# bkomuves/plonky2-verifier

Measured on AMD Instinct MI355X. Metric: Plonky2 proofs verified/sec (std config, 28 FRI queries) at 1/2/4/8 MI355X, higher is better.
Workload: dtype u64 (Goldilocks mod-p integer)

## Files before the change

### plonky2-verifier_amd/csrc/api_selftest.cpp

```cpp
#include "api_internal.hpp"
#include "kernels.h"

extern "C" {

static int selftest_field(int op, const uint64_t* a, const uint64_t* b, uint64_t* out, size_t n) {
  static const size_t kB[9] = {0, 0, 0, 0, 0, 1, 1, 12, 1}, kIn[9] = {2, 4, 1, 2, 4, 1, 2, 0, 0}, kOut[9] = {5, 2, 1, 2, 4, 1, 2, 2, 2};
  const size_t bw = kB[op - 12], wo = kOut[op - 12];
  size_t w = kIn[op - 12];
  if (bw && !b) return fail(P2V_E_ARG, "bad op / null argument");
  if (op == 17 && b[0] > 32) return fail(P2V_E_ARG, "pow_root: k > 32");
  if (op == 18 && b[0] > 0xFFFFFFFFull) return fail(P2V_E_ARG, "epow_u: e >= 2^32");
  if (op == 19) {
    w = (size_t)b[0];
    bool ok = b[0] >= 2 && b[0] <= (1u << 20) && b[1] <= 5;
    for (int k = 0; k < 5 && ok; k++) ok = b[2 + k] <= b[0] && b[7 + k] <= b[0] - b[2 + k];
    if (!ok) return fail(P2V_E_ARG, "reduce_powers: segment table outside the item");
  }
  if (op == 20) {
    if (b[0] < 1 || b[0] > 8) return fail(P2V_E_ARG, "fold: arity bits outside 1..8");
    w = 2 + (2u << b[0]);
  }
  if (n > (size_t)INT32_MAX - 64) return fail(P2V_E_ARG, "too many items");
  if (n == 0) return P2V_OK;
  Circuit C;
  C.arities = {1, 2, 3, 4, 5, 6, 7, 8};
  C.step_depth.assign(8, 0); C.L.step_evals.assign(8, 0); C.L.step_path.assign(8, 0);
  DevCircuit d{};
  fill_scalars(C, d);
  DevBuf da, db, dout, dtw;
#define SCK(x) HCK_AS("p2v_selftest", x)
  SCK(da.alloc(n * w * 8)); SCK(db.alloc(bw * 8)); SCK(dout.alloc(n * wo * 8));
  SCK(upload(dtw, fri_twiddles(C), d.twiddles));
  SCK(hipMemcpy(da.p, a, n * w * 8, hipMemcpyHostToDevice));
  if (bw) SCK(hipMemcpy(db.p, b, bw * 8, hipMemcpyHostToDevice));
  d.soa = (const uint64_t*)da.p; d.words = (int64_t)w; d.wstride = 1; d.tiled = 0;
  d.n = (int32_t)n; d.B = (int32_t)((n + 63) / 64 * 64);
  hipLaunchKernelGGL(k_selftest_field, dim3((unsigned)((n + 255) / 256)), dim3(256), 0, 0, op, d, (const uint64_t*)db.p, (uint64_t*)dout.p);
  SCK(hipGetLastError());
  SCK(hipMemcpy(out, dout.p, n * wo * 8, hipMemcpyDeviceToHost));
#undef SCK
  return P2V_OK;
}

static int selftest_prog(int device, const uint64_t* a, const uint64_t* b, uint64_t* out, size_t n) {
  if (!b) return fail(P2V_E_ARG, "bad op / null argument");
  if (b[0] > (1u << 20) || b[1] > (1u << 20)) return fail(P2V_E_ARG, "gate program rows beyond this build's limits");
  if (n > (size_t)INT32_MAX - 64) return fail(P2V_E_ARG, "too many items");
  const int64_t nw = (int64_t)b[0], nc = (int64_t)b[1];
  GateProgram g;
  std::vector<uint64_t> low;
  try {
    if (b[2] != P2V_WORDS_GATE_MAGIC) throw ParseError("gate program: bad magic / version");
    if (b[3] > (uint64_t)P2V_GATE_PROGRAM_MAX_INSTRS) throw CircuitError("gate program beyond this build's limits (instructions)");
    g = decode_gate_program(b + 2, gate_program_extent(b + 2, 2 + 3 * (size_t)b[3]));
    if (g.max_wire >= nw || g.max_const >= nc) throw CircuitError("(Array.!): gate program reads beyond the row");
    if (g.max_pih >= 4) throw CircuitError("(!!): gate program reads a public-inputs-hash word beyond 4");
    if (lower_gate_program(g, &low) > P2V_GATE_PROGRAM_MAX_LIVE) throw CircuitError("gate program beyond this build's limits (values alive at once)");
  } catch (const std::exception& e) { return fail(P2V_E_ARG, std::string("selftest op 21: ") + e.what()); }
  const int ndev = p2v_device_count();
  if (ndev == 0) return fail(P2V_E_NODEVICE, "no HIP device");
  if (device < 0 || device >= ndev) return fail(P2V_E_ARG, "bad device index");
  if (n == 0 || g.num_commits == 0) return P2V_OK;
  HCK(hipSetDevice(device));
  const size_t w = (size_t)(2 * (nw + nc) + 4), wo = 2 * (size_t)g.num_commits;
  DevCircuit d{};
  d.prog_pih = 2 * (nw + nc);
  d.o_wires = 0; d.o_const = 2 * nw;
  d.words = (int64_t)w; d.wstride = 1; d.tiled = 0;
  d.n = (int32_t)n; d.B = (int32_t)((n + 63) / 64 * 64);
  DevBuf da, dout, dprog;
#define SCK(x) HCK_AS("p2v_selftest", x)
  SCK(da.alloc(n * w * 8)); SCK(dout.alloc(n * wo * 8));
  SCK(upload(dprog, low, d.gprog));
  SCK(hipMemcpy(da.p, a, n * w * 8, hipMemcpyHostToDevice));
  d.soa = (const uint64_t*)da.p;
  hipLaunchKernelGGL(k_selftest_prog, dim3((unsigned)((n + 63) / 64)), dim3(64), 0, 0, d, (uint64_t*)dout.p, g.num_commits);
  SCK(hipGetLastError());
  SCK(hipMemcpy(out, dout.p, n * wo * 8, hipMemcpyDeviceToHost));
#undef SCK
  return P2V_OK;
}

int p2v_selftest(int device, int op, const uint64_t* a, const uint64_t* b, uint64_t* out, size_t n) {
  const bool needs_b = op == 0 || op == 3 || op == 4 || op == 6;
  if (op < 0 || op > 21 || op == 11 || (n && (!a || !out || (needs_b && !b)))) return fail(P2V_E_ARG, "bad op / null argument");
  if (op == 21) return selftest_prog(device, a, b, out, n);
  const int ndev = p2v_device_count();
  if (ndev == 0) return fail(P2V_E_NODEVICE, "no HIP device");
  if (device < 0 || device >= ndev) return fail(P2V_E_ARG, "bad device index");
  if (op < 12 && n == 0) return P2V_OK;
  HCK(hipSetDevice(device));
  if (op >= 12) return selftest_field(op, a, b, out, n);
  const bool scalar = op == 0 || op == 3 || op == 5 || op == 6 || op == 7 || op == 8;
  const size_t w = scalar ? 1 : 12, wo = op == 6 ? 2 : w;
  const size_t bw = op == 4 ? 24 : scalar && needs_b ? n : 2;
  DevBuf da, db, dout;
#define SCK(x) HCK_AS("p2v_selftest", x)
  SCK(da.alloc(n * w * 8)); SCK(db.alloc(bw * 8)); SCK(dout.alloc(n * wo * 8));
  SCK(hipMemcpy(da.p, a, n * w * 8, hipMemcpyHostToDevice));
  if (needs_b) SCK(hipMemcpy(db.p, b, bw * 8, hipMemcpyHostToDevice));
  if (op >= 9) {
    const int lanes = op == 9 ? 16 : 4;
    hipLaunchKernelGGL(k_selftest_forms, dim3((unsigned)((n * lanes + 255) / 256)), dim3(256), 0, 0, op, (const uint64_t*)da.p,
                       (uint64_t*)dout.p, (int64_t)n);
  } else {
    const size_t lanes = op == 8 ? 2 : 1;
    hipLaunchKernelGGL(k_selftest, dim3((unsigned)((n * lanes + 255) / 256)), dim3(256), 0, 0, op, (const uint64_t*)da.p,
                       (const uint64_t*)db.p, (uint64_t*)dout.p, (int64_t)n);
  }
  SCK(hipGetLastError());
  SCK(hipMemcpy(out, dout.p, n * wo * 8, hipMemcpyDeviceToHost));
#undef SCK
  return P2V_OK;
}

int p2v_count_mismatches(const int8_t* results, const int8_t* expect, size_t n, uint64_t* counters, void* stream) {
  if (!counters || (n && (!results || !expect))) return fail(P2V_E_ARG, "null argument");
  const unsigned blocks = n ? (unsigned)((n + 255) / 256) : 1;
  hipLaunchKernelGGL(k_count_mismatches, dim3(blocks), dim3(256), 0, (hipStream_t)stream, results, expect, (int64_t)n,
                     (unsigned long long*)counters);
  HCK(hipGetLastError());
  return P2V_OK;
}

int p2v_clock_probe(uint64_t* stamps, int nblocks, void* stream) {
  if (!stamps || nblocks <= 0) return fail(P2V_E_ARG, "null argument / no blocks");
  hipLaunchKernelGGL(k_clock_probe, dim3((unsigned)nblocks), dim3(64), 0, (hipStream_t)stream, (unsigned long long*)stamps);
  HCK(hipGetLastError());
  return P2V_OK;
}

}
```

### plonky2-verifier_amd/csrc/kernels.hip

```cpp
#include "leafhash.h"
#include "kernels.h"

using namespace p2d;
using gl::E;

__device__ __forceinline__ void leaf_hash_unit(const DevCircuit& c, int unit, int lane) {
  const int NPB = c.B >> 6;
  const int pb = unit % NPB, qt = unit / NPB;
  const int q = qt % c.Q, t = c.leaf_order[qt / c.Q];
  const int p = pb * 64 + lane;
  const int64_t base = c.q0 + (int64_t)q * c.qstride;
  int64_t off; int len;
  if (t < 4) { off = base + c.leaf[t]; len = c.lwidth[t]; }
  else { int s = t - 4; off = base + c.step_evals[s]; len = 2 << c.arity[s]; }
  uint64_t st[12];
  leaf_sponge(c, off, len, p, st);
  uint64_t* dst = c.leafdig + ((int64_t)(q * c.T + t) * 4) * c.B + p;
#pragma unroll
  for (int i = 0; i < 4; i++) dst[(int64_t)i * c.B] = st[i];
}

template <int D>
__device__ __forceinline__ uint64_t row_up(uint64_t v, bool plus) {
  const uint32_t lo = (uint32_t)v, hi = (uint32_t)(v >> 32);
// ... 461 lines not shown
  const bool pow_ok = (resp & mask) == 0;
  int8_t st = 1;
  if (!eqs_ok || !pow_ok) st = 0;
  else {
    for (int q = 0; q < c.Q && st == 1; q++) {
      const uint8_t* mk = c.mk_ok + (int64_t)q * c.T * c.B + p;
      bool init_ok = mk[0] && mk[c.B] && mk[2 * (int64_t)c.B] && mk[3 * (int64_t)c.B];
      if (!init_ok) { st = -1; break; }
      const uint32_t bits = c.fri_bits[(int64_t)q * c.B + p];
      for (int s = 0; s < c.S; s++) {
        if (!mk[(int64_t)(4 + s) * c.B]) { st = -2; break; }
        if (!((bits >> s) & 1u)) { st = -3; break; }
      }
      if (st != 1) break;
      if (!((bits >> 31) & 1u)) st = 0;
    }
  }
  if (c.key_id && c.key_id[p] >= (uint32_t)c.nkeys) st = -6;
  results[p] = st;
  if (trace) {
    uint64_t* tr = trace + (int64_t)p * trace_words;
    const int r = c.r, S = c.S, Q = c.Q;
    int64_t k = 0;
    for (int64_t w = 0; w < CH_QIDX(c) + Q; w++) tr[k++] = chal(c, w, p);
    for (int i = 0; i < 4 * r; i++) tr[k++] = c.van[(int64_t)(1 + i) * c.B + p];
    for (int j = 0; j < 3; j++)
      for (int q = 0; q < Q; q++) {
        const uint64_t* qv = c.qvals + (int64_t)q * 6 * c.B + p;
        tr[k++] = qv[(int64_t)(2 * j) * c.B];
        tr[k++] = qv[(int64_t)(2 * j + 1) * c.B];
      }
    tr[k++] = (uint64_t)(eqs_ok ? 1 : 0) | ((uint64_t)(pow_ok ? 1 : 0) << 1);
    for (int i = 0; i < r * c.nluts; i++) tr[k++] = c.lutre[(int64_t)i * c.B + p];
    (void)S;
  }
}

extern "C" __global__ void __launch_bounds__(256) k_selftest(int op, const uint64_t* a, const uint64_t* b, uint64_t* out, int64_t n) {
  const int64_t i = (int64_t)blockIdx.x * blockDim.x + threadIdx.x;
  if (op == 8) {
#if defined(__HIP_DEVICE_COMPILE__)
    const int64_t item = i >> 1;
    const uint64_t x = lp::sbox_u(a[item < n ? item : n - 1], (int)(i & 1));
    if (item < n && !(i & 1)) out[item] = gl::canon(x);
#endif
    return;
  }
  if (i >= n) return;
  if (op >= 5 && op <= 7) {
#if defined(__HIP_DEVICE_COMPILE__)
    if (op == 5) { uint64_t x = a[i]; p2::dv::sbox_n<1>(&x); out[i] = gl::canon(x); }
    else if (op == 6) { uint64_t x[2] = {a[i], b[i]}; p2::dv::sbox_n<2>(x); out[2 * i] = gl::canon(x[0]); out[2 * i + 1] = gl::canon(x[1]); }
    else out[i] = gl::canon(lp::sbox(a[i]));
#endif
  } else if (op == 0) {
    out[i] = gl::mul(a[i], b[i]);
  } else if (op == 3) {
#if defined(__HIP_DEVICE_COMPILE__)
    out[i] = gl::canon(gl::mul_nc_dev_v<2>(a[i], b[i]));
#endif
  } else if (op == 4) {
#if defined(__HIP_DEVICE_COMPILE__)
    uint64_t st[12], t[12], kl[12], kh[12];
#pragma unroll
    for (int k = 0; k < 12; k++) { st[k] = a[12 * i + k]; kl[k] = b[k]; kh[k] = b[12 + k]; }
    p2::dv::mds_group<0>(st, t, kl, kh);
    p2::dv::mds_group<4>(st, t, kl, kh);
    p2::dv::mds_group<8>(st, t, kl, kh);
#pragma unroll
    for (int k = 0; k < 12; k++) out[12 * i + k] = t[k];
#endif
  } else {
    uint64_t s[12];
#pragma unroll
    for (int k = 0; k < 12; k++) s[k] = op == 2 && k >= 8 ? 0 : a[12 * i + k];
    if (op == 1) p2::permute_dev(s);
    else p2::permute_dev(s, true, 1);
#pragma unroll
    for (int k = 0; k < 12; k++) out[12 * i + k] = op == 2 && k >= 4 ? 0 : s[k];
  }
}

extern "C" __global__ void __launch_bounds__(256) k_selftest_forms(int op, const uint64_t* a, uint64_t* out, int64_t n) {
  __shared__ TLdsAny T;
  tlds_fill_form(T, op == 9 ? 16 : 4);
  const int lanes = op == 9 ? 16 : 4;
  const int64_t g = (int64_t)blockIdx.x * 256 + threadIdx.x;
  const int64_t item = g / lanes, src = item < n ? item : n - 1;
  const int t = (int)(g % lanes);
  const uint64_t* s = a + 12 * src;
  uint64_t* o = out + 12 * item;
  if (op == 9) {
    lp::Row LR;
    lp::init(LR, T.l, threadIdx.x);
    const uint64_t x = lp::permute(LR.L < 12 ? s[LR.L] : 0, LR, T.l);
    if (item < n && LR.L < 12) o[LR.L] = x;
  } else {
    uint64_t x[3] = {s[3 * t], s[3 * t + 1], s[3 * t + 2]};
    qp::permute(x, t, T.q);
    if (item < n) for (int k = 0; k < 3; k++) o[3 * t + k] = x[k];
  }
}

extern "C" __global__ void __launch_bounds__(256) k_selftest_field(int op, DevCircuit c, const uint64_t* b, uint64_t* out) {
  const int64_t i = (int64_t)blockIdx.x * blockDim.x + threadIdx.x;
  const int p = (int)i;
  const bool live = i < c.n;
  if (op == 12) {
    const uint64_t x = ld(c, 0, p), y = ld(c, 1, p);
    const uint64_t r[5] = {gl::add(x, y), gl::sub(x, y), gl::neg(x), gl::mul_small(x, 7), gl::mul_small(x, (uint32_t)y)};
    if (live) for (int k = 0; k < 5; k++) out[5 * i + k] = r[k];
  } else if (op == 13) {
    const E x = lde(c, 0, p), y = lde(c, 2, p);
    const E r = gl::eeq(x, y) ? gl::esqr(x) : gl::emul(x, y);
    if (live) { out[2 * i] = r.a; out[2 * i + 1] = r.b; }
  } else if (op == 14) {
    const uint64_t r = inv_chain(ld(c, 0, p));
    if (live) out[i] = r;
  } else if (op == 15) {
    const E r = einv(lde(c, 0, p));
    if (live) { out[2 * i] = r.a; out[2 * i + 1] = r.b; }
  } else if (op == 16) {
    E iu, iv;
    einv2(lde(c, 0, p), lde(c, 2, p), iu, iv);
    if (live) { out[4 * i] = iu.a; out[4 * i + 1] = iu.b; out[4 * i + 2] = iv.a; out[4 * i + 3] = iv.b; }
  } else if (op == 17) {
    const uint64_t r = pow_root(c, (int)b[0], (uint32_t)ld(c, 0, p));
    if (live) out[i] = r;
  } else if (op == 18) {
    const E r = epow_u(lde(c, 0, p), (uint32_t)b[0]);
    if (live) { out[2 * i] = r.a; out[2 * i + 1] = r.b; }
  } else if (op == 19) {
    Segs S;
    S.ns = (int)b[1];
    for (int k = 0; k < 5; k++) { S.off[k] = (int64_t)b[2 + k]; S.n[k] = (int)b[7 + k]; }
    const E alpha = lde(c, 0, p);
    E ap[9];
    alpha_powers(alpha, ap);
    const E r = reduce_powers(c, S, p, alpha, ap);
    if (live) { out[2 * i] = r.a; out[2 * i + 1] = r.b; }
  } else if (op == 20) {
    const int ab = (int)b[0];
    const E r = fold_step(c, ab - 1, ab, 2, p, lde(c, 0, p));
    if (live) { out[2 * i] = r.a; out[2 * i + 1] = r.b; }
  }
}
```

### plonky2-verifier_amd/csrc/merkle.hip

```cpp
#include "leafhash.h"
#include "kernels.h"

using namespace p2d;

__device__ __forceinline__ uint32_t entry_pack(int t, int q, int p) { return (uint32_t)t << 27 | (uint32_t)q << 22 | (uint32_t)p; }
__device__ __forceinline__ void entry_unpack(uint32_t id, int& t, int& q, int& p) {
  t = (int)(id >> 27); q = (int)((id >> 22) & 31); p = (int)(id & 0x3FFFFFu);
}
__device__ __forceinline__ uint32_t plan_pack(int e, int owner, bool same_leaf, int root) {
  return (uint32_t)e | (uint32_t)owner << 4 | (uint32_t)same_leaf << 9 | (uint32_t)root << 10;
}
__device__ __forceinline__ int plan_e(uint32_t pw) { return (int)(pw & 15); }
__device__ __forceinline__ int plan_owner(uint32_t pw) { return (int)((pw >> 4) & 31); }
__device__ __forceinline__ bool plan_same_leaf(uint32_t pw) { return (pw >> 9) & 1; }
__device__ __forceinline__ int plan_root(uint32_t pw) { return (int)((pw >> 10) & 31); }
__device__ __forceinline__ uint8_t& mk_at(const DevCircuit& c, int t, int q, int p) { return c.mk_ok[(int64_t)(q * c.T + t) * c.B + p]; }

#ifndef P2V_MERKLE_WAVES
#define P2V_MERKLE_WAVES 6
#endif
#if P2V_MERKLE_WAVES > 0
#define P2V_MERKLE_ATTR __attribute__((amdgpu_waves_per_eu(P2V_MERKLE_WAVES)))
#else
#define P2V_MERKLE_ATTR
#endif
__device__ __forceinline__ void tree_path(const DevCircuit& c, int t, int q, int p, int& depth, int64_t& poff, uint32_t& idx) {
  const int64_t base = c.q0 + (int64_t)q * c.qstride;
  idx = (uint32_t)chal(c, CH_QIDX(c) + q, p);
  if (t < 4) { depth = c.depth0; poff = base + c.path[t]; }
  else {
    const int s = t - 4;
    int sh = 0;
    for (int j = 0; j <= s; j++) sh += c.arity[j];
    idx >>= sh; depth = c.step_depth[s]; poff = base + c.step_path[s];
  }
}
__device__ __forceinline__ void load_leafdig(const DevCircuit& c, int t, int q, int p, uint64_t (&cur)[4]) {
  const uint64_t* src = c.leafdig + ((int64_t)(q * c.T + t) * 4) * c.B + p;
#pragma unroll
  for (int i = 0; i < 4; i++) cur[i] = src[(int64_t)i * c.B];
}
__device__ __forceinline__ uint64_t cap_root(const DevCircuit& c, int t, uint32_t ci, int i, int p) {
  if (t == 0) return c.key_id ? lane_key(c, p)[ci * 4 + i] : c.cs_cap[ci * 4 + i];
  if (t == 1) return ld(c, c.wcap + ci * 4 + i, p);
  if (t == 2) return ld(c, c.zcap + ci * 4 + i, p);
  if (t == 3) return ld(c, c.qcap + ci * 4 + i, p);
  return ld(c, c.ccaps + (int64_t)(t - 4) * 4 * c.cap_len + ci * 4 + i, p);
}

__device__ __forceinline__ void merkle_level(uint64_t (&cur)[4], const uint64_t (&sib)[4], bool odd) {
  uint64_t st[12];
#pragma unroll
  for (int i = 0; i < 4; i++) { st[i] = odd ? sib[i] : cur[i]; st[4 + i] = odd ? cur[i] : sib[i]; st[8 + i] = 0; }
  p2::permute_dev(st, true, 1);
#pragma unroll
  for (int i = 0; i < 4; i++) cur[i] = st[i];
}
struct NoNode { __device__ __forceinline__ void operator()(int) const {} };
template <class F = NoNode>
__device__ __forceinline__ void lane_climb(const DevCircuit& c, int64_t poff, int l0, int l1, int p, uint64_t (&cur)[4], uint32_t& idx, F node = F{}) {
  for (int l = l0; l < l1; l++) {
    uint64_t sib[4];
#pragma unroll
    for (int i = 0; i < 4; i++) sib[i] = ld(c, poff + 4 * l + i, p);
    node(l);
    merkle_level(cur, sib, idx & 1u);
    idx >>= 1;
  }
}
__device__ __forceinline__ bool cap_ok(const DevCircuit& c, int t, uint32_t idx, const uint64_t (&cur)[4], int p) {
  bool ok = idx < (uint32_t)c.cap_len;
  const uint32_t ci = ok ? idx : 0;
#pragma unroll
  for (int i = 0; i < 4; i++) ok = ok && (cap_root(c, t, ci, i, p) == cur[i]);
  return ok;
}

__device__ __forceinline__ uint64_t row_climb(const DevCircuit& c, int64_t poff, int l0, int depth, int p, const lp::Row& LR, const lp::TLdsL& TL,
                                              uint64_t cur, uint32_t& idx) {
  const int L = LR.L;
  for (int l = l0; l < depth; l++) {
    const uint64_t sib = L < 8 ? ld(c, poff + 4 * l + (L & 3), p) : 0;
    const uint64_t c0 = rp::get_word(cur, 0), c1 = rp::get_word(cur, 1), c2 = rp::get_word(cur, 2), c3 = rp::get_word(cur, 3);
    const uint64_t cb = L == 4 ? c0 : L == 5 ? c1 : L == 6 ? c2 : c3;
    const bool odd = idx & 1u;
    const uint64_t x = L < 4 ? (odd ? sib : cur) : L < 8 ? (odd ? cb : sib) : 0;
    cur = lp::permute(x, LR, TL);
    idx >>= 1;
  }
  return cur;
}
__device__ __forceinline__ bool row_cap_ok(const DevCircuit& c, int t, uint32_t idx, uint64_t cur, int p, int L) {
  const bool ok = idx < (uint32_t)c.cap_len;
  const uint32_t ci = ok ? idx : 0;
  uint64_t root = 0;
  if (L < 4) root = cap_root(c, t, ci, L, p);
  const uint64_t eq = (L >= 4 || root == cur) ? 1 : 0;
  return ok && (rp::get_word(eq, 0) & rp::get_word(eq, 1) & rp::get_word(eq, 2) & rp::get_word(eq, 3));
}

__device__ __forceinline__ bool path_ok(const DevCircuit& c, int t, int q, int p) {
  int depth; int64_t poff; uint32_t idx;
  tree_path(c, t, q, p, depth, poff, idx);
  uint64_t cur[4];
  load_leafdig(c, t, q, p, cur);
  lane_climb(c, poff, 0, depth, p, cur, idx);
  return cap_ok(c, t, idx, cur, p);
}
__device__ __forceinline__ void merkle_unit(const DevCircuit& c) {
  const int lane = threadIdx.x & 63;
  const int unit = blockIdx.x * 4 + (threadIdx.x >> 6);
  const int NPB = c.B >> 6;
  if (unit >= c.Q * c.T * NPB) return;
  const int pb = unit % NPB, qt = unit / NPB;
  const int q = qt % c.Q, t = c.merkle_order[qt / c.Q];
  const int p = pb * 64 + lane;
  mk_at(c, t, q, p) = path_ok(c, t, q, p) ? 1 : 0;
}
extern "C" __global__ void __launch_bounds__(256) P2V_MERKLE_ATTR k_merkle(DevCircuit c) { merkle_unit(c); }

#define P2V_CSE_CSTRIDE 16
__device__ __forceinline__ void class_shape(const DevCircuit& c, int cls, int& sh, int& depth) {
  sh = 0; depth = c.depth0;
  if (cls > 0) { for (int j = 0; j < cls; j++) sh += c.arity[j]; depth = c.step_depth[cls - 1]; }
}
__device__ __forceinline__ int tree_class(int t) { return t < 4 ? 0 : t - 3; }
__device__ __forceinline__ int64_t plan_at(const DevCircuit& c, int t, int q, int p) { return ((int64_t)tree_class(t) * c.Q + q) * c.B + p; }
extern "C" __global__ void __launch_bounds__(64 * P2V_PLAN_WAVES) k_merkle_plan(DevCircuit c) {
  __shared__ int hist[P2V_CSE_MAX_DEPTH + 1], gbase[P2V_CSE_MAX_DEPTH + 1];
  const int lane = threadIdx.x & 63;
  const int unit = blockIdx.x * P2V_PLAN_WAVES + (threadIdx.x >> 6);
  const int NPB = c.B >> 6, ncls = 1 + c.S;
  const int nb = c.depth0 + 1;
  if (threadIdx.x < (unsigned)nb) hist[threadIdx.x] = 0;
  __syncthreads();
  const bool unit_live = unit < ncls * c.Q * NPB;
  const int pb = unit % NPB, cq = unit / NPB;
  const int q = cq % c.Q, cls = unit_live ? cq / c.Q : 0;
  const int p = pb * 64 + lane;
  const bool live = unit_live && p < c.n;
  int sh, depth;
  class_shape(c, cls, sh, depth);
  const int ntr = cls == 0 ? 4 - c.kskip : 1, t0 = cls == 0 ? c.kskip : 3 + cls;
  int e = 0, loc = 0, cnt = 0;
  if (live) {
    const uint64_t* qi = c.chal + (int64_t)CH_QIDX(c) * c.B + p;
    const uint32_t me = (uint32_t)qi[(int64_t)q * c.B] >> sh;
    int minb = 64, owner = q, root = q;
    bool have_root = false;
    uint64_t fol = ~0ULL;
    for (int k0 = 0; k0 < c.Q; k0 += 4) {
      uint32_t ik[4];
#pragma unroll
      for (int u = 0; u < 4; u++) ik[u] = k0 + u < c.Q ? (uint32_t)qi[(int64_t)(k0 + u) * c.B] >> sh : me;
#pragma unroll
      for (int u = 0; u < 4; u++) {
        const int k = k0 + u;
        if (k >= c.Q) break;
        const uint32_t x = me ^ ik[u];
        const int b = x ? 32 - __clz(x) : 0;
        if (!have_root && b <= depth) { root = k; have_root = true; }
        if (k < q) {
          if (b < minb) { minb = b; owner = k; }
        } else if (k > q && b >= 1 && b <= depth) {
          const int sl = 5 * (b - 1);
          if (((fol >> sl) & 31) == 31) fol ^= (uint64_t)(31 ^ k) << sl;
        }
      }
    }
    e = minb - 1 >= depth ? depth : (minb >= 1 ? minb - 1 : 0);
    if (e < depth) fol |= ~0ULL << (5 * e);
    const int64_t pi = ((int64_t)cls * c.Q + q) * c.B + p;
    c.mplan[pi] = plan_pack(e, owner, minb == 0, root);
    c.mfol[pi] = fol;
    for (int tt = 0; tt < ntr; tt++) {
      c.mbadq[((int64_t)(t0 + tt) * c.Q + q) * c.B + p] = 0;
      mk_at(c, t0 + tt, q, p) = 0;
    }
  }
  uint64_t todo = __ballot(live);
  while (todo) {
    const int lead = __ffsll((unsigned long long)todo) - 1;
    const int eb = __shfl(e, lead);
    const uint64_t grp = __ballot(live && e == eb);
    const int n = __popcll(grp);
    int off = 0;
    if (lane == lead) off = atomicAdd(&hist[eb], n * ntr);
    off = __shfl(off, lead);
    if (live && e == eb) { loc = off + __popcll(grp & ((1ULL << lane) - 1)); cnt = n; }
// ... 335 lines not shown
```

### plonky2-verifier_amd/csrc/poseidon.h

```cpp
#pragma once
#include "gl.h"
#include "poseidon_constants.h"
#include "pasm.h"

namespace p2 {

static constexpr uint32_t MDS_CIRC[12] = {17, 15, 41, 16, 2, 28, 13, 13, 39, 18, 34, 20};
static constexpr uint32_t MDS_DIAG0 = 8;
__host__ __device__ constexpr uint32_t mds_coeff(int i, int j) {
  return MDS_CIRC[((j - i) % 12 + 12) % 12] + (i == j && i == 0 ? MDS_DIAG0 : 0);
}

#if defined(__HIPCC__)
static __constant__ uint64_t c_round_constants[360] = P2V_ALL_ROUND_CONSTANTS_INIT;
static __constant__ uint64_t c_fast_first_rc[12] = P2V_FAST_PARTIAL_FIRST_ROUND_CONSTANT_INIT;
static __constant__ uint64_t c_fast_rc[22] = P2V_FAST_PARTIAL_ROUND_CONSTANTS_INIT;
static __constant__ uint64_t c_fast_vs[22 * 11] = P2V_FAST_PARTIAL_ROUND_VS_INIT;
static __constant__ uint64_t c_fast_w_hats[22 * 11] = P2V_FAST_PARTIAL_ROUND_W_HATS_INIT;
static __constant__ uint64_t c_fast_init_matrix[11 * 11] = P2V_FAST_PARTIAL_ROUND_INITIAL_MATRIX_INIT;
#endif
static const uint64_t h_round_constants[360] = P2V_ALL_ROUND_CONSTANTS_INIT;

__host__ __device__ __forceinline__ uint64_t add_nc(uint64_t a, uint64_t b) {
  uint64_t s = a + b;
// ... 68 lines not shown
struct RcSplit { uint64_t lo[31 * 12], hi[31 * 12]; };
__host__ __device__ constexpr RcSplit make_rc_split() {
  RcSplit t{};
  constexpr uint64_t rc[360] = P2V_ALL_ROUND_CONSTANTS_INIT;
  for (int k = 0; k < 360; k++) { t.lo[k] = rc[k] & 0xFFFFFFFFull; t.hi[k] = rc[k] >> 32; }
  return t;
}
struct ZhConst { uint64_t z[4]; };
__host__ __device__ constexpr uint64_t cx_mul(uint64_t a, uint64_t b) { return (uint64_t)(((unsigned __int128)a * b) % gl::P); }
__host__ __device__ constexpr ZhConst make_zh() {
  ZhConst t{};
  constexpr uint64_t rc[360] = P2V_ALL_ROUND_CONSTANTS_INIT;
  for (int i = 0; i < 4; i++) {
    const uint64_t x = rc[8 + i] % gl::P, x2 = cx_mul(x, x), x3 = cx_mul(x2, x), x4 = cx_mul(x2, x2);
    t.z[i] = cx_mul(x3, x4);
  }
  return t;
}
static __constant__ RcSplit c_rc_split = make_rc_split();
static __constant__ ZhConst c_zh = make_zh();
struct ZrcSplit { uint64_t lo[12], hi[12]; };
__host__ __device__ constexpr ZrcSplit make_zrc() {
  ZrcSplit t{};
  constexpr uint64_t rc[360] = P2V_ALL_ROUND_CONSTANTS_INIT;
  const ZhConst z = make_zh();
  for (int i = 0; i < 12; i++) {
    unsigned __int128 a = rc[12 + i] % gl::P;
    for (int j = 8; j < 12; j++) a += (unsigned __int128)mds_coeff(i, j) * z.z[j - 8];
    const uint64_t k = (uint64_t)(a % gl::P);
    t.lo[i] = k & 0xFFFFFFFFull;
    t.hi[i] = k >> 32;
  }
  return t;
}
static __constant__ ZrcSplit c_zrc = make_zrc();
#endif

struct PBlock {
  uint32_t cf[14][16];
  uint64_t dlo[16], dhi[16];
};
static constexpr int PM_NB = 6;
static constexpr int PM_SCHED[PM_NB] = {4, 4, 4, 4, 4, 2};
struct PMTab { PBlock b[PM_NB]; };
__host__ __device__ constexpr uint64_t cx_addp(uint64_t a, uint64_t b) { return (uint64_t)(((unsigned __int128)a + b) % gl::P); }
__host__ __device__ constexpr uint64_t cx_mulp(uint64_t a, uint64_t b) { return (uint64_t)(((unsigned __int128)a * b) % gl::P); }
__host__ __device__ constexpr int pm_rounds() { int n = 0; for (int b = 0; b < PM_NB; b++) n += PM_SCHED[b]; return n; }
static_assert(pm_rounds() == 22, "the merge schedule must cover the 22 partial rounds");
struct PMAlg { uint64_t G[5][12][12], H[5][5][12]; };
__host__ __device__ constexpr PMAlg pm_alg() {
  PMAlg A{};
  for (int i = 0; i < 12; i++)
    for (int j = 0; j < 12; j++) A.G[1][i][j] = mds_coeff(i, j);
  for (int k = 2; k <= 4; k++) {
    for (int i = 0; i < 12; i++) {
      for (int j = 0; j < 12; j++) {
        uint64_t a = 0;
        for (int l = 1; l < 12; l++) a += mds_coeff(i, l) * A.G[k - 1][l][j];
        A.G[k][i][j] = a;
      }
      for (int m = 2; m < k; m++) {
        uint64_t a = 0;
        for (int l = 1; l < 12; l++) a += mds_coeff(i, l) * A.H[k - 1][m][l];
        A.H[k][m][i] = a;
      }
      A.H[k][k][i] = mds_coeff(i, 0);
    }
  }
  return A;
}
struct PMD { uint64_t d[5][12]; };
__host__ __device__ constexpr PMD pm_d(int r, int D) {
  PMD R{};
  constexpr uint64_t rc[360] = P2V_ALL_ROUND_CONSTANTS_INIT;
  for (int i = 0; i < 12; i++) R.d[1][i] = rc[12 * (r + 1) + i] % gl::P;
  for (int k = 2; k <= D; k++)
    for (int i = 0; i < 12; i++) {
      uint64_t a = rc[12 * (r + k) + i] % gl::P;
      for (int l = 1; l < 12; l++) a = cx_addp(a, cx_mulp(mds_coeff(i, l), R.d[k - 1][l]));
      R.d[k][i] = a;
    }
  return R;
}
__host__ __device__ constexpr PMTab make_pm() {
  PMTab T{};
  const PMAlg A = pm_alg();
  int r = 4;
  for (int b = 0; b < PM_NB; b++) {
    const int D = PM_SCHED[b];
    const PMD dd = pm_d(r, D);
    PBlock& B = T.b[b];
    for (int k = 1; k < D; k++) { B.dlo[k - 1] = dd.d[k][0] & 0xFFFFFFFFull; B.dhi[k - 1] = dd.d[k][0] >> 32; }
    for (int k = 2; k < D; k++) {
      for (int j = 0; j < 12; j++) B.cf[k - 2][j] = (uint32_t)A.G[k][0][j];
      for (int m = 2; m < k; m++) B.cf[k - 2][12 + m - 2] = (uint32_t)A.H[k][m][0];
    }
    for (int i = 0; i < 12; i++) {
      for (int j = 0; j < 12; j++) B.cf[2 + i][j] = (uint32_t)A.G[D][i][j];
      for (int m = 2; m < D; m++) B.cf[2 + i][12 + m - 2] = (uint32_t)A.H[D][m][i];
      B.dlo[4 + i] = dd.d[D][i] & 0xFFFFFFFFull;
      B.dhi[4 + i] = dd.d[D][i] >> 32;
    }
    r += D;
  }
  return T;
}
#if defined(__HIPCC__)
static __constant__ PMTab c_pm = make_pm();
#endif

#if defined(__HIP_DEVICE_COMPILE__)
namespace dv {
template <uint32_t C>
__device__ __forceinline__ uint64_t madk(uint32_t a, uint64_t acc) {
  uint64_t d;
  asm("v_mad_u64_u32 %0, s[94:95], %1, %2, %3" : "=v"(d) : "v"(a), "n"(C), "v"(acc) : "s94", "s95");
  return d;
}
template <uint32_t C>
__device__ __forceinline__ uint64_t madk_s(uint32_t a, uint64_t acc) {
  uint64_t d;
  asm("v_mad_u64_u32 %0, s[94:95], %1, %2, %3" : "=v"(d) : "v"(a), "n"(C), "s"(acc) : "s94", "s95");
  return d;
}
__device__ __forceinline__ uint64_t reduce_rows(uint64_t al, uint64_t ah) {
  using namespace gl::ax;
  uint64_t c1, c2;
  const uint64_t t = madm1_co((uint32_t)(ah >> 32), al, c1);
  const uint32_t rh = add_co((uint32_t)(t >> 32), (uint32_t)ah, c1);
  uint64_t r = ((uint64_t)rh << 32) | (uint32_t)t;
  if (__builtin_expect(c1 != 0, 0)) r = madm1_co(mask_1(c1), r, c2);
  return r;
}
template <int I, int J, int E = 12>
__device__ __forceinline__ void mds_acc(const uint64_t* s, uint64_t& al, uint64_t& ah) {
  if constexpr (J < E) {
    constexpr uint32_t C = mds_coeff(I, J);
    al = madk<C>((uint32_t)s[J], al);
    ah = madk<C>((uint32_t)(s[J] >> 32), ah);
    mds_acc<I, J + 1, E>(s, al, ah);
  }
}
template <int I, int NW = 12>
__device__ __forceinline__ void row_unfixed(const uint64_t* s, const uint64_t* kl, const uint64_t* kh, uint64_t& r, uint64_t& c) {
  using namespace gl::ax;
  constexpr uint32_t C = mds_coeff(I, 0);
  uint64_t al = madk_s<C>((uint32_t)s[0], kl[I]);
  uint64_t ah = madk_s<C>((uint32_t)(s[0] >> 32), kh[I]);
  mds_acc<I, 1, NW>(s, al, ah);
  uint64_t c0;
  const uint64_t t = madm1_co((uint32_t)(ah >> 32), al, c0);
  const uint32_t rh = add_co((uint32_t)(t >> 32), (uint32_t)ah, c);
  r = ((uint64_t)rh << 32) | (uint32_t)t;
}
template <int I, int NW = 12>
__device__ __forceinline__ void mds_group(const uint64_t* s, uint64_t* t, const uint64_t* kl, const uint64_t* kh) {
  using namespace gl::ax;
  uint64_t r0, r1, r2, r3, c0, c1, c2, c3, d;
  row_unfixed<I, NW>(s, kl, kh, r0, c0);
  row_unfixed<I + 1, NW>(s, kl, kh, r1, c1);
  row_unfixed<I + 2, NW>(s, kl, kh, r2, c2);
  row_unfixed<I + 3, NW>(s, kl, kh, r3, c3);
  if (__builtin_expect((c0 | c1 | c2 | c3) != 0, 0)) {
    r0 = madm1_co(mask_1(c0), r0, d);
    r1 = madm1_co(mask_1(c1), r1, d);
    r2 = madm1_co(mask_1(c2), r2, d);
    r3 = madm1_co(mask_1(c3), r3, d);
  }
  t[I] = r0; t[I + 1] = r1; t[I + 2] = r2; t[I + 3] = r3;
}
template <int I, int E>
__device__ __forceinline__ void mds_rows(const uint64_t* s, uint64_t* t, const uint64_t* kl, const uint64_t* kh) {
  if constexpr (I < E) {
    constexpr uint32_t C = mds_coeff(I, 0);
    uint64_t al = madk_s<C>((uint32_t)s[0], kl[I]);
    uint64_t ah = madk_s<C>((uint32_t)(s[0] >> 32), kh[I]);
    mds_acc<I, 1>(s, al, ah);
    t[I] = reduce_rows(al, ah);
    mds_rows<I + 1, E>(s, t, kl, kh);
  }
}
template <int N>
__device__ __forceinline__ void sbox_n(uint64_t* x) {
  uint64_t x2[N], x3[N], x4[N], n2[N], n3[N], n4[N];
#pragma unroll
  for (int i = 0; i < N; i++) x2[i] = gl::mul_nc_part(x[i], x[i], n2[i]);
  uint64_t any = 0;
#pragma unroll
  for (int i = 0; i < N; i++) any |= n2[i];
  if (__builtin_expect(any != 0, 0)) {
#pragma unroll
// ... 9 lines not shown
    for (int i = 0; i < N; i++) { x3[i] = gl::mul_fix_neg(x3[i], n3[i]); x4[i] = gl::mul_fix_neg(x4[i], n4[i]); }
  }
#pragma unroll
  for (int i = 0; i < N; i++) x[i] = gl::mul_nc_part(x3[i], x4[i], n2[i]);
  any = 0;
#pragma unroll
  for (int i = 0; i < N; i++) any |= n2[i];
  if (__builtin_expect(any != 0, 0)) {
#pragma unroll
    for (int i = 0; i < N; i++) x[i] = gl::mul_fix_neg(x[i], n2[i]);
  }
}
static constexpr int SBOX_ILP = 2;
template <int I, int E>
__device__ __forceinline__ void sbox_range(uint64_t* s) {
  if constexpr (I < E) {
    constexpr int K = (E - I) < SBOX_ILP ? (E - I) : SBOX_ILP;
    sbox_n<K>(s + I);
    sbox_range<I + K, E>(s);
  }
}
__device__ __forceinline__ uint64_t sbox_one(uint64_t x) {
  sbox_n<1>(&x);
  return x;
}
__device__ __forceinline__ void round_pp(uint64_t* s, uint64_t* t, int r, bool zh0, int g) {
  sbox_range<0, 8>(s);
  if (zh0) {
#pragma unroll
    for (int i = 8; i < 12; i++) s[i] = c_zh.z[i - 8];
  } else {
    sbox_range<8, 12>(s);
  }
  const uint64_t* kl = c_rc_split.lo + 12 * (r + 1);
  const uint64_t* kh = c_rc_split.hi + 12 * (r + 1);
  if (g & 1) mds_group<0>(s, t, kl, kh);
  if (g & 2) mds_group<4>(s, t, kl, kh);
  if (g & 4) mds_group<8>(s, t, kl, kh);
}

__device__ __forceinline__ void round0_zh(uint64_t* s, uint64_t* t) {
  sbox_range<0, 8>(s);
  mds_group<0, 8>(s, t, c_zrc.lo, c_zrc.hi);
  mds_group<4, 8>(s, t, c_zrc.lo, c_zrc.hi);
  mds_group<8, 8>(s, t, c_zrc.lo, c_zrc.hi);
}

__device__ __forceinline__ uint64_t madv(uint32_t a, uint32_t c, uint64_t acc) {
  uint64_t d;
  asm("v_mad_u64_u32 %0, s[94:95], %1, %2, %3" : "=v"(d) : "v"(a), "s"(c), "v"(acc) : "s94", "s95");
  return d;
}
__device__ __forceinline__ uint64_t reduce_t(uint64_t al, uint64_t ah) {
  using namespace gl::ax;
  uint64_t c0, c1, c2;
  const uint64_t t = madm1_co((uint32_t)(ah >> 32), al, c0);
  const uint32_t rh = add_co((uint32_t)(t >> 32), (uint32_t)ah, c1);
  return madm1_co(mask_1(c1), ((uint64_t)rh << 32) | (uint32_t)t, c2);
}
__device__ __forceinline__ uint64_t reduce_w(uint64_t al, uint64_t ah) {
  using namespace gl::ax;
  uint64_t c0, c1, c2;
  const uint32_t lh = add_co((uint32_t)(al >> 32), (uint32_t)ah, c0);
  const uint32_t hi = addc0((uint32_t)(ah >> 32), c0);
  const uint64_t r = madm1_co(hi, ((uint64_t)lh << 32) | (uint32_t)al, c1);
  return madm1_co(mask_1(c1), r, c2);
}
template <uint32_t CI, int NH>
__device__ __forceinline__ void prow(const uint64_t* s, const uint64_t* yh, uint64_t yn, const uint32_t* cf,
                                     uint64_t dl, uint64_t dh, uint64_t& al, uint64_t& ah) {
  al = madk_s<CI>((uint32_t)yn, dl);
  ah = madk_s<CI>((uint32_t)(yn >> 32), dh);
#pragma unroll
  for (int j = 0; j < 12; j++) {
    al = madv((uint32_t)s[j], cf[j], al);
    ah = madv((uint32_t)(s[j] >> 32), cf[j], ah);
  }
#pragma unroll
  for (int m = 0; m < NH; m++) {
    al = madv((uint32_t)yh[m], cf[12 + m], al);
    ah = madv((uint32_t)(yh[m] >> 32), cf[12 + m], ah);
  }
}
template <int I>
__device__ __forceinline__ void pblock4_rows(const uint64_t* s, const uint64_t* y, uint64_t* t, const PBlock& B) {
  if constexpr (I < 12) {
    uint64_t al, ah;
    prow<mds_coeff(I, 0), 2>(s, y + 2, y[4], B.cf[2 + I], B.dlo[4 + I], B.dhi[4 + I], al, ah);
    t[I] = reduce_w(al, ah);
    pblock4_rows<I + 1>(s, y, t, B);
  }
}
template <int I>
__device__ __forceinline__ void prow2_unfixed(const uint64_t* s, uint64_t y2, const PBlock& B, uint64_t& r, uint64_t& c) {
  using namespace gl::ax;
  uint64_t al, ah, c0;
  prow<mds_coeff(I, 0), 0>(s, nullptr, y2, B.cf[2 + I], B.dlo[4 + I], B.dhi[4 + I], al, ah);
  const uint64_t tt = madm1_co((uint32_t)(ah >> 32), al, c0);
  const uint32_t rh = add_co((uint32_t)(tt >> 32), (uint32_t)ah, c);
  r = ((uint64_t)rh << 32) | (uint32_t)tt;
}
template <int I>
__device__ __forceinline__ void pblock2_group(const uint64_t* s, uint64_t y2, uint64_t* t, const PBlock& B) {
  using namespace gl::ax;
  uint64_t r0, r1, r2, r3, c0, c1, c2, c3, d;
  prow2_unfixed<I>(s, y2, B, r0, c0);
  prow2_unfixed<I + 1>(s, y2, B, r1, c1);
  prow2_unfixed<I + 2>(s, y2, B, r2, c2);
  prow2_unfixed<I + 3>(s, y2, B, r3, c3);
  if (__builtin_expect((c0 | c1 | c2 | c3) != 0, 0)) {
    r0 = madm1_co(mask_1(c0), r0, d);
    r1 = madm1_co(mask_1(c1), r1, d);
    r2 = madm1_co(mask_1(c2), r2, d);
    r3 = madm1_co(mask_1(c3), r3, d);
  }
  t[I] = r0; t[I + 1] = r1; t[I + 2] = r2; t[I + 3] = r3;
}
template <int D>
__device__ __forceinline__ void pblock(uint64_t* s, uint64_t* t, const PBlock& B) {
  static_assert(D == 2 || D == 4, "PM_SCHED holds blocks of 4 and 2");
  uint64_t y[D + 1];
  s[0] = sbox_one(s[0]);
  {
    uint64_t al = madk_s<mds_coeff(0, 0)>((uint32_t)s[0], B.dlo[0]);
    uint64_t ah = madk_s<mds_coeff(0, 0)>((uint32_t)(s[0] >> 32), B.dhi[0]);
    mds_acc<0, 1>(s, al, ah);
    y[2] = sbox_one(reduce_rows(al, ah));
  }
  if constexpr (D == 4) {
    uint64_t al, ah;
    prow<mds_coeff(0, 0), 0>(s, nullptr, y[2], B.cf[0], B.dlo[1], B.dhi[1], al, ah);
    y[3] = sbox_one(reduce_rows(al, ah));
    prow<mds_coeff(0, 0), 1>(s, y + 2, y[3], B.cf[1], B.dlo[2], B.dhi[2], al, ah);
    y[4] = sbox_one(reduce_t(al, ah));
    pblock4_rows<0>(s, y, t, B);
  } else {
    pblock2_group<0>(s, y[2], t, B);
    pblock2_group<4>(s, y[2], t, B);
    pblock2_group<8>(s, y[2], t, B);
  }
}
}

template <bool FOLD = true>
__device__ __forceinline__ void permute_dev(uint64_t s[12], bool zh = false, int gm = 7) {
  uint64_t t[12];
  int fl = __builtin_amdgcn_readfirstlane((zh ? 8 : 0) | gm);
  asm("" : "+s"(fl));
  zh = fl & 8;
  gm = fl & 7;
  const uint64_t* rc0 = c_round_constants;
  asm volatile("" : "+s"(rc0));
#pragma unroll
  for (int i = 0; i < 8; i++) s[i] = add_nc(s[i], rc0[i]);
  int k0 = 0;
  if constexpr (FOLD) if (zh) {
    dv::round0_zh(s, t);
    dv::round_pp(t, s, 1, false, 7);
    k0 = 1;
  }
  if (!zh) {
#pragma unroll
    for (int i = 8; i < 12; i++) s[i] = add_nc(s[i], rc0[i]);
  }
#pragma unroll 1
  for (int k = k0; k < 4; k++) {
    const int r = k < 2 ? 2 * k : 22 + 2 * k;
    dv::round_pp(s, t, r, zh && k == 0, 7);
    dv::round_pp(t, s, r + 1, false, k == 3 ? gm : 7);
    if (k == 1) {
#pragma unroll 1
      for (int b = 0; b < 4; b += 2) {
        dv::pblock<4>(s, t, c_pm.b[b]);
        dv::pblock<4>(t, s, c_pm.b[b + 1]);
      }
      dv::pblock<4>(s, t, c_pm.b[4]);
      dv::pblock<2>(t, s, c_pm.b[5]);
    }
  }
  if (gm & 1) {
#pragma unroll
    for (int i = 0; i < 4; i++) s[i] = gl::canon(s[i]);
  }
  if (gm & 2) {
#pragma unroll
    for (int i = 4; i < 8; i++) s[i] = gl::canon(s[i]);
  }
  if (gm & 4) {
#pragma unroll
    for (int i = 8; i < 12; i++) s[i] = gl::canon(s[i]);
  }
}
#elif defined(__HIPCC__)
template <bool FOLD = true>
__device__ void permute_dev(uint64_t s[12], bool zh = false, int gm = 7);
namespace dv { template <uint32_t C> __device__ uint64_t madk(uint32_t a, uint64_t acc); }
#endif

__host__ __device__ __forceinline__ void permute(uint64_t s[12]) {
#if defined(__HIP_DEVICE_COMPILE__)
  permute_dev(s);
#else
  for (int r = 0; r < 4; r++) full_round(s, r);
  for (int r = 4; r < 26; r++) partial_round(s, r);
  for (int r = 26; r < 30; r++) full_round(s, r);
  P2_UNROLL
  for (int i = 0; i < 12; i++) s[i] = gl::canon(s[i]);
#endif
}

}
```

Measured before the change: 1.612 million.

## Fold last pre-partial full round into a depth-3 leading partial block

Adds an alternative Poseidon permutation schedule (LEAD) where the final full round before the partial rounds is merged with the first two partial rounds into a depth-3 precomputed block. The remaining 20 partial rounds run as five depth-4 blocks, replacing the previous 4,4,4,4,4,2 schedule. It becomes the default for permute_dev, while the Merkle leaf climb explicitly keeps the old path. This aims to cut per-permutation MDS/multiply work and block overhead, at the cost of a second constant table and an extra output buffer. A selftest op for the leading block is added.

```diff
diff --git a/plonky2-verifier_amd/csrc/api_selftest.cpp b/plonky2-verifier_amd/csrc/api_selftest.cpp
--- a/plonky2-verifier_amd/csrc/api_selftest.cpp
+++ b/plonky2-verifier_amd/csrc/api_selftest.cpp
@@ -83,14 +83,14 @@
 
 int p2v_selftest(int device, int op, const uint64_t* a, const uint64_t* b, uint64_t* out, size_t n) {
   const bool needs_b = op == 0 || op == 3 || op == 4 || op == 6;
-  if (op < 0 || op > 21 || op == 11 || (n && (!a || !out || (needs_b && !b)))) return fail(P2V_E_ARG, "bad op / null argument");
+  if (op < 0 || op > 22 || op == 11 || (n && (!a || !out || (needs_b && !b)))) return fail(P2V_E_ARG, "bad op / null argument");
   if (op == 21) return selftest_prog(device, a, b, out, n);
   const int ndev = p2v_device_count();
   if (ndev == 0) return fail(P2V_E_NODEVICE, "no HIP device");
   if (device < 0 || device >= ndev) return fail(P2V_E_ARG, "bad device index");
-  if (op < 12 && n == 0) return P2V_OK;
+  if ((op < 12 || op == 22) && n == 0) return P2V_OK;
   HCK(hipSetDevice(device));
-  if (op >= 12) return selftest_field(op, a, b, out, n);
+  if (op >= 12 && op <= 20) return selftest_field(op, a, b, out, n);
   const bool scalar = op == 0 || op == 3 || op == 5 || op == 6 || op == 7 || op == 8;
   const size_t w = scalar ? 1 : 12, wo = op == 6 ? 2 : w;
   const size_t bw = op == 4 ? 24 : scalar && needs_b ? n : 2;
@@ -100,7 +100,7 @@
   SCK(hipMemcpy(da.p, a, n * w * 8, hipMemcpyHostToDevice));
   if (needs_b) SCK(hipMemcpy(db.p, b, bw * 8, hipMemcpyHostToDevice));
   if (op >= 9) {
-    const int lanes = op == 9 ? 16 : 4;
+    const size_t lanes = op == 9 ? 16 : op == 10 ? 4 : 1;
     hipLaunchKernelGGL(k_selftest_forms, dim3((unsigned)((n * lanes + 255) / 256)), dim3(256), 0, 0, op, (const uint64_t*)da.p,
                        (uint64_t*)dout.p, (int64_t)n);
   } else {
diff --git a/plonky2-verifier_amd/csrc/kernels.hip b/plonky2-verifier_amd/csrc/kernels.hip
--- a/plonky2-verifier_amd/csrc/kernels.hip
+++ b/plonky2-verifier_amd/csrc/kernels.hip
@@ -567,6 +567,19 @@
 }
 
 extern "C" __global__ void __launch_bounds__(256) k_selftest_forms(int op, const uint64_t* a, uint64_t* out, int64_t n) {
+  if (op == 22) {
+#if defined(__HIP_DEVICE_COMPILE__)
+    const int64_t i = (int64_t)blockIdx.x * 256 + threadIdx.x;
+    if (i >= n) return;
+    uint64_t u[12], t[12];
+#pragma unroll
+    for (int k = 0; k < 12; k++) u[k] = a[12 * i + k];
+    p2::dv::pblock<3, true>(u, t, p2::c_pf.lead);
+#pragma unroll
+    for (int k = 0; k < 12; k++) out[12 * i + k] = gl::canon(t[k]);
+#endif
+    return;
+  }
   __shared__ TLdsAny T;
   tlds_fill_form(T, op == 9 ? 16 : 4);
   const int lanes = op == 9 ? 16 : 4;
diff --git a/plonky2-verifier_amd/csrc/merkle.hip b/plonky2-verifier_amd/csrc/merkle.hip
--- a/plonky2-verifier_amd/csrc/merkle.hip
+++ b/plonky2-verifier_amd/csrc/merkle.hip
@@ -48,23 +48,24 @@
   return ld(c, c.ccaps + (int64_t)(t - 4) * 4 * c.cap_len + ci * 4 + i, p);
 }
 
+template <bool LEAD = true>
 __device__ __forceinline__ void merkle_level(uint64_t (&cur)[4], const uint64_t (&sib)[4], bool odd) {
   uint64_t st[12];
 #pragma unroll
   for (int i = 0; i < 4; i++) { st[i] = odd ? sib[i] : cur[i]; st[4 + i] = odd ? cur[i] : sib[i]; st[8 + i] = 0; }
-  p2::permute_dev(st, true, 1);
+  p2::permute_dev<true, LEAD>(st, true, 1);
 #pragma unroll
   for (int i = 0; i < 4; i++) cur[i] = st[i];
 }
 struct NoNode { __device__ __forceinline__ void operator()(int) const {} };
-template <class F = NoNode>
+template <class F = NoNode, bool LEAD = true>
 __device__ __forceinline__ void lane_climb(const DevCircuit& c, int64_t poff, int l0, int l1, int p, uint64_t (&cur)[4], uint32_t& idx, F node = F{}) {
   for (int l = l0; l < l1; l++) {
     uint64_t sib[4];
 #pragma unroll
     for (int i = 0; i < 4; i++) sib[i] = ld(c, poff + 4 * l + i, p);
     node(l);
-    merkle_level(cur, sib, idx & 1u);
+    merkle_level<LEAD>(cur, sib, idx & 1u);
     idx >>= 1;
   }
 }
@@ -104,7 +105,7 @@
   tree_path(c, t, q, p, depth, poff, idx);
   uint64_t cur[4];
   load_leafdig(c, t, q, p, cur);
-  lane_climb(c, poff, 0, depth, p, cur, idx);
+  lane_climb<NoNode, false>(c, poff, 0, depth, p, cur, idx);
   return cap_ok(c, t, idx, cur, p);
 }
 __device__ __forceinline__ void merkle_unit(const DevCircuit& c) {
diff --git a/plonky2-verifier_amd/csrc/poseidon.h b/plonky2-verifier_amd/csrc/poseidon.h
--- a/plonky2-verifier_amd/csrc/poseidon.h
+++ b/plonky2-verifier_amd/csrc/poseidon.h
@@ -174,31 +174,46 @@
     }
   return R;
 }
+__host__ __device__ constexpr PBlock pm_block(const PMAlg& A, int r, int D) {
+  PBlock B{};
+  const PMD dd = pm_d(r, D);
+  for (int k = 1; k < D; k++) { B.dlo[k - 1] = dd.d[k][0] & 0xFFFFFFFFull; B.dhi[k - 1] = dd.d[k][0] >> 32; }
+  for (int k = 2; k < D; k++) {
+    for (int j = 0; j < 12; j++) B.cf[k - 2][j] = (uint32_t)A.G[k][0][j];
+    for (int m = 2; m < k; m++) B.cf[k - 2][12 + m - 2] = (uint32_t)A.H[k][m][0];
+  }
+  for (int i = 0; i < 12; i++) {
+    for (int j = 0; j < 12; j++) B.cf[2 + i][j] = (uint32_t)A.G[D][i][j];
+    for (int m = 2; m < D; m++) B.cf[2 + i][12 + m - 2] = (uint32_t)A.H[D][m][i];
+    B.dlo[4 + i] = dd.d[D][i] & 0xFFFFFFFFull;
+    B.dhi[4 + i] = dd.d[D][i] >> 32;
+  }
+  return B;
+}
 __host__ __device__ constexpr PMTab make_pm() {
   PMTab T{};
   const PMAlg A = pm_alg();
   int r = 4;
   for (int b = 0; b < PM_NB; b++) {
-    const int D = PM_SCHED[b];
-    const PMD dd = pm_d(r, D);
-    PBlock& B = T.b[b];
-    for (int k = 1; k < D; k++) { B.dlo[k - 1] = dd.d[k][0] & 0xFFFFFFFFull; B.dhi[k - 1] = dd.d[k][0] >> 32; }
-    for (int k = 2; k < D; k++) {
-      for (int j = 0; j < 12; j++) B.cf[k - 2][j] = (uint32_t)A.G[k][0][j];
-      for (int m = 2; m < k; m++) B.cf[k - 2][12 + m - 2] = (uint32_t)A.H[k][m][0];
-    }
-    for (int i = 0; i < 12; i++) {
-      for (int j = 0; j < 12; j++) B.cf[2 + i][j] = (uint32_t)A.G[D][i][j];
-      for (int m = 2; m < D; m++) B.cf[2 + i][12 + m - 2] = (uint32_t)A.H[D][m][i];
-      B.dlo[4 + i] = dd.d[D][i] & 0xFFFFFFFFull;
-      B.dhi[4 + i] = dd.d[D][i] >> 32;
-    }
-    r += D;
-  }
+    T.b[b] = pm_block(A, r, PM_SCHED[b]);
+    r += PM_SCHED[b];
+  }
+  return T;
+}
+static constexpr int PF_LEAD = 2;
+static constexpr int PF_NB = 5;
+static_assert(PF_LEAD + 4 * PF_NB == 22, "the schedule must cover the 22 partial rounds");
+struct PFTab { PBlock lead; PBlock b[PF_NB]; };
+__host__ __device__ constexpr PFTab make_pf() {
+  PFTab T{};
+  const PMAlg A = pm_alg();
+  T.lead = pm_block(A, 3, PF_LEAD + 1);
+  for (int b = 0; b < PF_NB; b++) T.b[b] = pm_block(A, 4 + PF_LEAD + 4 * b, 4);
   return T;
 }
 #if defined(__HIPCC__)
 static __constant__ PMTab c_pm = make_pm();
+static __constant__ PFTab c_pf = make_pf();
 #endif
 
 #if defined(__HIP_DEVICE_COMPILE__)
@@ -374,13 +389,13 @@
     ah = madv((uint32_t)(yh[m] >> 32), cf[12 + m], ah);
   }
 }
-template <int I>
-__device__ __forceinline__ void pblock4_rows(const uint64_t* s, const uint64_t* y, uint64_t* t, const PBlock& B) {
+template <int D, int I>
+__device__ __forceinline__ void pblock_rows(const uint64_t* s, const uint64_t* y, uint64_t* t, const PBlock& B) {
   if constexpr (I < 12) {
     uint64_t al, ah;
-    prow<mds_coeff(I, 0), 2>(s, y + 2, y[4], B.cf[2 + I], B.dlo[4 + I], B.dhi[4 + I], al, ah);
-    t[I] = reduce_w(al, ah);
-    pblock4_rows<I + 1>(s, y, t, B);
+    prow<mds_coeff(I, 0), D - 2>(s, y + 2, y[D], B.cf[2 + I], B.dlo[4 + I], B.dhi[4 + I], al, ah);
+    t[I] = D == 4 ? reduce_w(al, ah) : reduce_t(al, ah);
+    pblock_rows<D, I + 1>(s, y, t, B);
   }
 }
 template <int I>
@@ -408,33 +423,32 @@
   }
   t[I] = r0; t[I + 1] = r1; t[I + 2] = r2; t[I + 3] = r3;
 }
-template <int D>
+template <int D, bool LEAD = false>
 __device__ __forceinline__ void pblock(uint64_t* s, uint64_t* t, const PBlock& B) {
-  static_assert(D == 2 || D == 4, "PM_SCHED holds blocks of 4 and 2");
-  uint64_t y[D + 1];
-  s[0] = sbox_one(s[0]);
-  {
-    uint64_t al = madk_s<mds_coeff(0, 0)>((uint32_t)s[0], B.dlo[0]);
-    uint64_t ah = madk_s<mds_coeff(0, 0)>((uint32_t)(s[0] >> 32), B.dhi[0]);
-    mds_acc<0, 1>(s, al, ah);
-    y[2] = sbox_one(reduce_rows(al, ah));
-  }
-  if constexpr (D == 4) {
-    uint64_t al, ah;
-    prow<mds_coeff(0, 0), 0>(s, nullptr, y[2], B.cf[0], B.dlo[1], B.dhi[1], al, ah);
-    y[3] = sbox_one(reduce_rows(al, ah));
-    prow<mds_coeff(0, 0), 1>(s, y + 2, y[3], B.cf[1], B.dlo[2], B.dhi[2], al, ah);
-    y[4] = sbox_one(reduce_t(al, ah));
-    pblock4_rows<0>(s, y, t, B);
-  } else {
+  static_assert(LEAD ? D == 3 : D == 2 || D == 4, "blocks of 4 and 2, and the leading unit at depth 3");
+  uint64_t y[D + 1], al, ah;
+  if constexpr (!LEAD) s[0] = sbox_one(s[0]);
+  al = madk_s<mds_coeff(0, 0)>((uint32_t)s[0], B.dlo[0]);
+  ah = madk_s<mds_coeff(0, 0)>((uint32_t)(s[0] >> 32), B.dhi[0]);
+  mds_acc<0, 1>(s, al, ah);
+  y[2] = sbox_one(reduce_rows(al, ah));
+  if constexpr (D == 2) {
     pblock2_group<0>(s, y[2], t, B);
     pblock2_group<4>(s, y[2], t, B);
     pblock2_group<8>(s, y[2], t, B);
-  }
-}
-}
-
-template <bool FOLD = true>
+  } else {
+    prow<mds_coeff(0, 0), 0>(s, nullptr, y[2], B.cf[0], B.dlo[1], B.dhi[1], al, ah);
+    y[3] = sbox_one(reduce_rows(al, ah));
+    if constexpr (D == 4) {
+      prow<mds_coeff(0, 0), 1>(s, y + 2, y[3], B.cf[1], B.dlo[2], B.dhi[2], al, ah);
+      y[4] = sbox_one(reduce_t(al, ah));
+    }
+    pblock_rows<D, 0>(s, y, t, B);
+  }
+}
+}
+
+template <bool FOLD = true, bool LEAD = true>
 __device__ __forceinline__ void permute_dev(uint64_t s[12], bool zh = false, int gm = 7) {
   uint64_t t[12];
   int fl = __builtin_amdgcn_readfirstlane((zh ? 8 : 0) | gm);
@@ -455,36 +469,57 @@
 #pragma unroll
     for (int i = 8; i < 12; i++) s[i] = add_nc(s[i], rc0[i]);
   }
+  uint64_t o[12];
+  if constexpr (LEAD) {
 #pragma unroll 1
-  for (int k = k0; k < 4; k++) {
-    const int r = k < 2 ? 2 * k : 22 + 2 * k;
-    dv::round_pp(s, t, r, zh && k == 0, 7);
-    dv::round_pp(t, s, r + 1, false, k == 3 ? gm : 7);
-    if (k == 1) {
+    for (int k = k0; k < 3; k++) {
+      dv::round_pp(s, t, k < 2 ? 2 * k : 23 + 2 * k, zh && k == 0, 7);
+      if (k == 1) {
+        dv::sbox_range<0, 12>(t);
+        dv::pblock<3, true>(t, s, c_pf.lead);
 #pragma unroll 1
-      for (int b = 0; b < 4; b += 2) {
-        dv::pblock<4>(s, t, c_pm.b[b]);
-        dv::pblock<4>(t, s, c_pm.b[b + 1]);
+        for (int b = 0; b < 4; b += 2) {
+          dv::pblock<4>(s, t, c_pf.b[b]);
+          dv::pblock<4>(t, s, c_pf.b[b + 1]);
+        }
+        dv::pblock<4>(s, t, c_pf.b[4]);
       }
-      dv::pblock<4>(s, t, c_pm.b[4]);
-      dv::pblock<2>(t, s, c_pm.b[5]);
+      dv::round_pp(t, s, k == 0 ? 1 : 24 + 2 * k, false, 7);
     }
-  }
+    dv::round_pp(s, o, 29, false, gm);
+  } else {
+#pragma unroll 1
+    for (int k = k0; k < 4; k++) {
+      const int r = k < 2 ? 2 * k : 22 + 2 * k;
+      dv::round_pp(s, t, r, zh && k == 0, 7);
+      dv::round_pp(t, s, r + 1, false, k == 3 ? gm : 7);
+      if (k == 1) {
+#pragma unroll 1
+        for (int b = 0; b < 4; b += 2) {
+          dv::pblock<4>(s, t, c_pm.b[b]);
+          dv::pblock<4>(t, s, c_pm.b[b + 1]);
+        }
+        dv::pblock<4>(s, t, c_pm.b[4]);
+        dv::pblock<2>(t, s, c_pm.b[5]);
+      }
+    }
+  }
+  const uint64_t* e = LEAD ? o : s;
   if (gm & 1) {
 #pragma unroll
-    for (int i = 0; i < 4; i++) s[i] = gl::canon(s[i]);
+    for (int i = 0; i < 4; i++) s[i] = gl::canon(e[i]);
   }
   if (gm & 2) {
 #pragma unroll
-    for (int i = 4; i < 8; i++) s[i] = gl::canon(s[i]);
+    for (int i = 4; i < 8; i++) s[i] = gl::canon(e[i]);
   }
   if (gm & 4) {
 #pragma unroll
-    for (int i = 8; i < 12; i++) s[i] = gl::canon(s[i]);
+    for (int i = 8; i < 12; i++) s[i] = gl::canon(e[i]);
   }
 }
 #elif defined(__HIPCC__)
-template <bool FOLD = true>
+template <bool FOLD = true, bool LEAD = true>
 __device__ void permute_dev(uint64_t s[12], bool zh = false, int gm = 7);
 namespace dv { template <uint32_t C> __device__ uint64_t madk(uint32_t a, uint64_t acc); }
 #endif
```

Result: faster. 1.633 million, median of 6 (+1.3%).
